# radygenomics/GROM

Measured on AMD Instinct MI355X. Metric: Mbases/sec scanned (whole genome) + VCF concordance vs ref, higher is better.
Workload: dtype int32

## Files before the change

grom_amd/csrc/ddecode.hip:

```cpp
#include <hip/hip_runtime.h>

#include <atomic>
#include <chrono>
#include <condition_variable>
#include <cstdio>
#include <cstdlib>
#include <cstring>
#include <mutex>
#include <vector>
#include <zlib.h>

#include "../../include/grom_amd.h"
#include "ddecode.h"
#include "inflate.h"

#define DD_LANES 64
#define DD_SLOTS 2
#define DD_RSLOTS 4

#define GI_E_BOUNDS 8
__device__ __forceinline__ bool dd_blk_inb(const DdBlock &b, int64_t o, int64_t comp_cap, int64_t out_cap) {
    return b.in_off >= 0 && b.in_off + (int64_t)b.in_len <= comp_cap && o >= 0 && b.out_len <= 65536u &&
           o + (int64_t)b.out_len <= out_cap;
}

__global__ void __launch_bounds__(DD_LANES, 2) k_inflate(const uint8_t *__restrict__ comp, int64_t comp_cap,
                                                      const DdBlock *__restrict__ blk, int64_t n_blk,
                                                      uint8_t *__restrict__ out, int64_t out_base, int64_t out_cap,
                                                      uint8_t *__restrict__ status, uint32_t *__restrict__ n_bad,
                                                      uint32_t *__restrict__ bounds, int only_tokcap) {
    extern __shared__ uint32_t dd_tab[];
    const int64_t j = (int64_t)blockIdx.x * DD_LANES + threadIdx.x;
    if (j >= n_blk) return;
    if (only_tokcap && status[j] != (uint8_t)GI_E_TOKCAP) return;
    const DdBlock b = blk[j];
    const int64_t o = b.out_off - out_base;
    if (!dd_blk_inb(b, o, comp_cap, out_cap)) {
        status[j] = (uint8_t)GI_E_BOUNDS;
        atomicAdd(n_bad, 1u);
        atomicOr(bounds, 1u);
        return;
    }
    const int rc = gi_inflate<DD_LANES>(comp + b.in_off, b.in_len, out + o, b.out_len, dd_tab, threadIdx.x);
    status[j] = (uint8_t)rc;
    if (rc) atomicAdd(n_bad, 1u);
}

__global__ void __launch_bounds__(DD_LANES, 2) k_huff(const uint8_t *__restrict__ comp, int64_t comp_cap,
                                                   const DdBlock *__restrict__ blk, int64_t n_blk,
                                                   uint8_t *__restrict__ out, int64_t out_base, int64_t out_cap,
                                                   uint32_t *__restrict__ tok, uint32_t *__restrict__ ntok,
                                                   uint32_t tokcap, uint8_t *__restrict__ status,
                                                   uint32_t *__restrict__ n_bad, uint32_t *__restrict__ bounds) {
    extern __shared__ uint32_t dd_tab[];
    const int64_t j = (int64_t)blockIdx.x * DD_LANES + threadIdx.x;
    if (j >= n_blk) return;
    const DdBlock b = blk[j];
    const int64_t o = b.out_off - out_base;
    if (!dd_blk_inb(b, o, comp_cap, out_cap)) {
        status[j] = (uint8_t)GI_E_BOUNDS;
        atomicAdd(n_bad, 1u);
        atomicOr(bounds, 1u);
        return;
    }
    const int rc = gi_tokens<DD_LANES>(comp + b.in_off, b.in_len, out + o, b.out_len, tok + (size_t)j * tokcap, tokcap,
                                       ntok + j, dd_tab, threadIdx.x);
    status[j] = (uint8_t)rc;
    if (rc && rc != GI_E_TOKCAP) atomicAdd(n_bad, 1u);
}

__device__ __forceinline__ uint32_t lz_wave_incl(uint32_t v, int lane) {
#pragma unroll
    for (int d = 1; d < 64; d <<= 1) {
        const uint32_t u = __shfl_up(v, d, 64);
        if (lane >= d) v += u;
    }
    return v;
}
__device__ __forceinline__ uint32_t lz_wave_min(uint32_t v) {
#pragma unroll
    for (int d = 32; d >= 1; d >>= 1) v = min(v, (uint32_t)__shfl_xor(v, d, 64));
    return v;
}

__global__ void __launch_bounds__(64) k_lz77(const DdBlock *__restrict__ blk, int64_t n_blk, uint8_t *__restrict__ out,
                                             int64_t out_base, const uint32_t *__restrict__ tok,
                                             const uint32_t *__restrict__ ntok, uint32_t tokcap,
                                             uint8_t *__restrict__ status, uint32_t *__restrict__ n_bad) {
    const int64_t j = blockIdx.x;
// ... 29 lines not shown
                bool blocked = false;
                for (uint64_t q = pm; q; q &= q - 1) {
                    const int jl = __builtin_ctzll(q);
                    const uint32_t mj = __builtin_amdgcn_readlane(m, jl);
                    const uint32_t ej = mj + __builtin_amdgcn_readlane(len, jl);
                    blocked = blocked || (mj < se && ej > src);
                }
                ready = pend && !blocked;
            }
            if (ready) {
                gi_match(dst, m, len, d);
                pend = false;
            }
            __builtin_amdgcn_fence(__ATOMIC_RELEASE, "workgroup");
            __builtin_amdgcn_fence(__ATOMIC_ACQUIRE, "workgroup");
        }
    }
    if (lane == 0 && (bad || obase != olen)) {
        status[j] = (uint8_t)GI_E_SIZE;
        atomicAdd(n_bad, 1u);
    }
}

__global__ void __launch_bounds__(DD_LANES) k_lz77_lane(const DdBlock *__restrict__ blk, int64_t n_blk,
                                                        uint8_t *__restrict__ out, int64_t out_base,
                                                        const uint32_t *__restrict__ tok,
                                                        const uint32_t *__restrict__ ntok, uint32_t tokcap,
                                                        uint8_t *__restrict__ status, uint32_t *__restrict__ n_bad) {
    const int64_t j = (int64_t)blockIdx.x * DD_LANES + threadIdx.x;
    if (j >= n_blk || status[j] != 0) return;
    const DdBlock b = blk[j];
    const int rc = gi_lz(tok + (size_t)j * tokcap, ntok[j], out + (b.out_off - out_base), b.out_len);
    if (rc) {
        status[j] = (uint8_t)rc;
        atomicAdd(n_bad, 1u);
    }
}

static uint32_t dd_tokcap() {
    static const uint32_t cap = [] {
        const char *e = getenv("GROM_INFLATE_TOKCAP");
        long v = e ? atol(e) : 0;
        if (v < 0) v = 0;
        if (v > 65536) v = 65536;
        return (uint32_t)(v & ~3L);
    }();
    return cap;
}

extern "C" size_t dd_inflate_tok_bytes(int64_t n_blk) {
    const uint32_t cap = dd_tokcap();
    return cap ? (size_t)n_blk * ((size_t)cap + 1) * 4 + 64 : 0;
}

extern "C" int dd_inflate_launch(hipStream_t st, const uint8_t *d_comp, int64_t comp_cap, const DdBlock *d_blk,
                                 int64_t n_blk, uint8_t *d_out, int64_t out_base, int64_t out_cap, uint8_t *d_status,
                                 uint32_t *d_bad, uint32_t *d_bounds, uint32_t *d_tok, size_t tok_bytes) {
    if (n_blk <= 0) return 0;
    const unsigned grid = (unsigned)((n_blk + DD_LANES - 1) / DD_LANES);
    static const int pad = getenv("GROM_INFLATE_LDS_PAD") ? atoi(getenv("GROM_INFLATE_LDS_PAD")) : 0;
    const uint32_t cap = dd_tokcap();
    if (cap == 0 || d_tok == nullptr || tok_bytes < dd_inflate_tok_bytes(n_blk)) {
        hipLaunchKernelGGL(k_inflate, dim3(grid), dim3(DD_LANES), GI_LANE_BYTES * DD_LANES + pad, st, d_comp, comp_cap,
                           d_blk, n_blk, d_out, out_base, out_cap, d_status, d_bad, d_bounds, 0);
        return hipGetLastError() == hipSuccess ? 0 : -1;
    }
    uint32_t *ntok = d_tok + (size_t)n_blk * cap;
    hipLaunchKernelGGL(k_huff, dim3(grid), dim3(DD_LANES), GI_LANE_BYTES * DD_LANES + pad, st, d_comp, comp_cap, d_blk,
                       n_blk, d_out, out_base, out_cap, d_tok, ntok, cap, d_status, d_bad, d_bounds);
    static const bool lane_lz = getenv("GROM_LZ_LANE") && atoi(getenv("GROM_LZ_LANE")) != 0;
    if (lane_lz)
        hipLaunchKernelGGL(k_lz77_lane, dim3(grid), dim3(DD_LANES), 0, st, d_blk, n_blk, d_out, out_base, d_tok, ntok,
                           cap, d_status, d_bad);
    else
        hipLaunchKernelGGL(k_lz77, dim3((unsigned)n_blk), dim3(64), 0, st, d_blk, n_blk, d_out, out_base, d_tok, ntok,
                           cap, d_status, d_bad);
    hipLaunchKernelGGL(k_inflate, dim3(grid), dim3(DD_LANES), GI_LANE_BYTES * DD_LANES + pad, st, d_comp, comp_cap,
                       d_blk, n_blk, d_out, out_base, out_cap, d_status, d_bad, d_bounds, 1);
    return hipGetLastError() == hipSuccess ? 0 : -1;
}

static uint16_t rd16(const uint8_t *p) { return (uint16_t)(p[0] | (p[1] << 8)); }
static uint32_t rd32(const uint8_t *p) {
    return (uint32_t)p[0] | (uint32_t)p[1] << 8 | (uint32_t)p[2] << 16 | (uint32_t)p[3] << 24;
}

extern "C" int64_t dd_block_table(const uint8_t *buf, int64_t len, DdBlock *out, int64_t cap, int64_t *out_bytes) {
    return dd_block_table_prefix(buf, len, out, cap, out_bytes, nullptr);
}

extern "C" int64_t dd_block_table_prefix(const uint8_t *buf, int64_t len, DdBlock *out, int64_t cap, int64_t *out_bytes,
                                         int64_t *consumed) {
    int64_t off = 0, n = 0, ob = 0;
    while (off < len) {
        if (off + 18 > len) {
            if (consumed) break;
            return -1;
        }
        const uint8_t *h = buf + off;
// ... 111 lines not shown
            inflateEnd(&zs);
            const bool same = zok ? (status[j] == 0 && memcmp(want.data(), got.data() + tab[j].out_off, tab[j].out_len) == 0)
                                  : status[j] != 0;
            if (!same) {
                if (bad < 5) fprintf(stderr, "device inflate: block %lld: zlib %d, device status %d\n", (long long)j, zrc,
                                     status[j]);
                bad++;
            }
        }
    }
done:
    if (n_blocks) *n_blocks = nb;
    if (bytes) *bytes = ob;
    if (e0) (void)hipEventDestroy(e0);
    if (e1) (void)hipEventDestroy(e1);
    if (st) (void)hipStreamDestroy(st);
    (void)hipFree(d_comp);
    (void)hipFree(d_out);
    (void)hipFree(d_status);
    (void)hipFree(d_blk);
    (void)hipFree(d_bad);
    (void)hipFree(d_tok);
    return bad;
}

#include <hipcub/hipcub.hpp>

#include "bamio.h"
#include "copystats.h"

namespace {

struct DBuf {
    void *p = nullptr;
    size_t cap = 0;
};

std::atomic<int64_t> g_dgrow_ns{0};

int dgrow(DBuf &b, size_t bytes, const char *what = nullptr) {
    if (bytes == 0) bytes = 16;
    if (b.cap >= bytes) return 0;
    const auto t0 = std::chrono::steady_clock::now();
    if (b.p) grom_dev_free(b.p, b.cap, GROM_DEVCAT_DECODE);
    b.p = nullptr;
    b.cap = 0;
// ... 1109 lines not shown
}

static int upload_run_tables(dd_ctx *c, const dd_run_req *q, hipStream_t st, char *err, int errlen) {
    const int64_t nblk = q->nblk, ns = q->n_starts;
    DBuf &rblk = c->rblk[q->slot], &rS = c->rS[q->slot];
    c->tab_gen[q->slot] = c->comp_gen[q->slot].load();
    DGROW(rblk, sizeof(DdBlock) * (size_t)(nblk + 1));
    DGROW(rS, sizeof(int64_t) * (size_t)(ns + 2));
    DCK(hipMemcpyAsync(rblk.p, q->blk, sizeof(DdBlock) * (size_t)nblk, hipMemcpyHostToDevice, st));
    DCK(hipMemcpyAsync(rS.p, q->starts, sizeof(int64_t) * (size_t)(ns + 1), hipMemcpyHostToDevice, st));
    return 0;
}

static int size_slot(RunSlot &r, const std::vector<Piece> &pcs, double rpb, char *err, int errlen) {
    int64_t mx_pb = 0, mx_blk = 0, mx_ch = 0, mx_oc = 0;
    for (const Piece &pc : pcs) {
        mx_pb = std::max(mx_pb, pc.pbytes);
        mx_blk = std::max(mx_blk, pc.bl - pc.bf + 2);
        mx_ch = std::max(mx_ch, pc.cb - pc.ca + 1);
        mx_oc = std::max(mx_oc, (int64_t)((double)pc.pbytes * rpb * 1.3) + 4096);
    }
    DGROW(r.U, (size_t)mx_pb + 64);
    DGROW(r.status, (size_t)mx_blk);
    DGROW(r.ccnt, sizeof(uint32_t) * (size_t)mx_ch);
    DGROW(r.cbase, sizeof(uint32_t) * (size_t)mx_ch);
    DGROW(r.misc, 256);
    DGROW(r.off, 8 * (size_t)(mx_oc + 1));
    size_t tb = 0;
    DCK(hipcub::DeviceScan::ExclusiveSum(nullptr, tb, (uint32_t *)nullptr, (uint32_t *)nullptr, (int)mx_ch, r.st));
    DGROW(r.tmp, tb);
    return 0;
}

__global__ void k_piece_summary(const uint32_t *__restrict__ cbase, const uint32_t *__restrict__ ccnt, int64_t nch,
                                uint32_t *__restrict__ rb, uint32_t *__restrict__ out) {
    if (threadIdx.x == 0) {
        out[0] = cbase[nch - 1];
        out[1] = ccnt[nch - 1];
        out[2] = rb[0];
        out[3] = rb[1];
        out[4] = rb[4];
        out[5] = rb[5];
    }
    __syncthreads();
    if (threadIdx.x < 16) rb[threadIdx.x] = 0;
}
// ... 507 lines not shown
```

grom_amd/csrc/inflate.h:

```cpp
#pragma once
#include <stdint.h>

#if defined(__HIP_DEVICE_COMPILE__)
#define GI_KEEP(x) asm volatile("" : "+v"(x))
#else
#define GI_KEEP(x) (void)0
#endif
#if defined(__HIPCC__)
#define GI_FN __host__ __device__ __forceinline__
#define GI_UNROLL _Pragma("unroll")
#else
#define GI_FN static inline
#define GI_UNROLL _Pragma("GCC unroll 16")
#endif

#define GI_T_LIT 0
#define GI_T_LITHI 72
#define GI_T_DIST 81
#ifndef GI_CLREG
#define GI_CLREG 0
#endif
#if GI_CLREG
#define GI_LANE_DWORDS 89
#else
// ... 104 lines not shown
        b.buf |= (uint64_t)b.q0 << b.cnt;
        b.q0 = b.q1;
        b.q1 = b.q2;
        b.q2 = b.q3;
        if (--b.kq == 0) {
            b.q0 = b.n0;
            b.q1 = b.n1;
            b.q2 = b.n2;
            b.q3 = b.n3;
            gi_ldq(b.wp, b.n0, b.n1, b.n2, b.n3);
            b.wp += 4;
            b.kq = 4;
        }
#else
        b.buf |= (uint64_t)b.nxt << b.cnt;
        b.nxt = gi_ldw(b.wp);
        b.wp++;
#endif
        b.cnt += 32;
        b.merged++;
    }
}

GI_FN uint32_t gi_bits(GiBits &b, int n) {
    const uint32_t v = (uint32_t)(b.buf & ((n >= 32) ? 0xffffffffull : ((1ull << n) - 1)));
    b.buf >>= n;
    b.cnt -= n;
    return v;
}

template <int LANES>
GI_FN uint8_t *gi_cell(uint32_t *tab, int t0, int r, int lane) {
    return (uint8_t *)(tab + (t0 + (r >> 2)) * LANES + lane) + (r & 3);
}

template <int N>
struct GiHuffT {
    uint32_t e[N + 1];
};
typedef GiHuffT<15> GiHuff;
typedef GiHuffT<7> GiHuffCL;

template <int N>
GI_FN int gi_code(GiHuffT<N> &h, uint32_t *cnt, int sh) {
    int32_t left = 1;
    uint32_t code = 0, off = 0;
GI_UNROLL
// ... 31 lines not shown
    }
}

template <int LANES, int N, bool HI, class Get>
GI_FN int gi_build(GiHuffT<N> &h, uint32_t *tab, int lane, int t0, int n, Get get) {
    uint32_t cnt[N + 1];
GI_UNROLL
    for (int l = 0; l <= N; l++) cnt[l] = 0;
    for (int i = 0; i < n; i++) {
        const uint32_t L = get(i);
GI_UNROLL
        for (int l = 1; l <= N; l++) cnt[l] += (L == (uint32_t)l) ? 1u : 0u;
    }
    const int rc = gi_code<N>(h, cnt, 0);
    if (rc) return rc;
    gi_clear_hi<LANES, HI>(tab, lane);
    for (int i = 0; i < n; i++) {
        const uint32_t L = get(i);
        if (L) gi_place<LANES, N, HI>(tab, t0, lane, cnt, 0, L, i);
    }
    return GI_OK;
}

template <int N>
GI_FN int gi_index(const GiBits &b, const GiHuffT<N> &h, int &L) {
    const uint32_t rev = gi_rev15((uint32_t)b.buf);
    const uint32_t key = rev << 16 | 0xffffu;
    L = 1;
    uint32_t bs = h.e[1];
GI_UNROLL
    for (int l = 1; l < N; l++) {
        const bool ge = key >= h.e[l];
        L += ge ? 1 : 0;
        bs = ge ? h.e[l + 1] : bs;
        GI_KEEP(bs);
    }
    if (key >= h.e[N]) return -1;
    return (int)(int16_t)(uint16_t)bs + (int)(rev >> (15 - L));
}

template <int LANES, int N, bool HI>
GI_FN int gi_lookup(const GiBits &b, const GiHuffT<N> &h, const uint32_t *tab, int lane, int t0, int &L) {
    const int idx = gi_index<N>(b, h, L);
    if (idx < 0) return -1;
    int s = *gi_cell<LANES>((uint32_t *)tab, t0, idx, lane);
    if (HI) s |= (int)((tab[(GI_T_LITHI + (idx >> 5)) * LANES + lane] >> (idx & 31)) & 1u) << 8;
    return s;
}

template <int LANES, int N, bool HI>
GI_FN int gi_decode(GiBits &b, const GiHuffT<N> &h, const uint32_t *tab, int lane, int t0) {
    int L;
    const int s = gi_lookup<LANES, N, HI>(b, h, tab, lane, t0, L);
    if (s < 0) return -1;
    b.buf >>= L;
    b.cnt -= L;
    return s;
}

GI_FN void gi_len_code(int s, int &base, int &extra) {
    if (s < 265) { base = s - 254; extra = 0; }
    else if (s < 285) { extra = (s - 261) >> 2; base = 3 + ((4 + ((s - 265) & 3)) << extra); }
    else { base = 258; extra = 0; }
}
GI_FN void gi_dist_code(int d, int &base, int &extra) {
    if (d < 4) { base = d + 1; extra = 0; }
    else { extra = (d >> 1) - 1; base = ((2 + (d & 1)) << extra) + 1; }
}

GI_FN int gi_cl_item(GiBits &b, int s, int prev, int &val) {
    if (s < 16) { val = s; return 1; }
    if (s == 16) { val = prev; return prev < 0 ? -1 : 3 + (int)gi_bits(b, 2); }
    val = 0;
    return s == 17 ? 3 + (int)gi_bits(b, 3) : 11 + (int)gi_bits(b, 7);
}

template <int LANES>
GI_FN int gi_fixed(GiHuff &lit, GiHuff &dist, uint32_t *tab, int lane) {
GI_UNROLL
    for (int w = 0; w < 72; w++) {
        uint32_t v = 0;
        for (int k = 0; k < 4; k++) {
            const int i = 4 * w + k;
            const int sym = i < 24 ? 256 + i : i < 168 ? i - 24 : i < 176 ? 280 + (i - 168) : 144 + (i - 176);
            v |= (uint32_t)(sym & 0xff) << (8 * k);
        }
        tab[(GI_T_LIT + w) * LANES + lane] = v;
    }
GI_UNROLL
    for (int w = 0; w < 9; w++) tab[(GI_T_LITHI + w) * LANES + lane] = w == 0 ? 0x00ffffffu : (w == 5 ? 0x0000ff00u : 0u);
GI_UNROLL
    for (int w = 0; w < 8; w++)
        tab[(GI_T_DIST + w) * LANES + lane] = (uint32_t)(4 * w) | (uint32_t)(4 * w + 1) << 8 | (uint32_t)(4 * w + 2) << 16 |
// ... 8 lines not shown

#ifndef GI_P2ONE
#define GI_P2ONE 1
#endif
struct GiHdr {
    GiHuffCL clh;
#if GI_CLREG
    uint32_t clt[4];
#endif
    int at;
    int n, ntot, nlit, prev, eob;
    int rl;
};

GI_FN void gi_seek(GiBits &b, const uint8_t *in, int pos) {
    const int mis = (int)((uintptr_t)in & 3);
    const int abs = mis * 8 + pos;
    b.sh0 = mis * 8;
    gi_start(b, (const uint32_t *)(in - mis), abs >> 5, abs & 31);
}

GI_FN int64_t gi_used(const GiBits &b) { return b.merged * 32 - b.sh0 - b.cnt; }

#if GI_CLREG
GI_FN int gi_build_cl(GiHdr &H, uint64_t cl) {
    uint32_t cnt[8];
GI_UNROLL
    for (int l = 0; l < 8; l++) cnt[l] = 0;
GI_UNROLL
    for (int i = 0; i < 19; i++) {
        const uint32_t L = (uint32_t)(cl >> (3 * i)) & 7u;
GI_UNROLL
        for (int l = 1; l <= 7; l++) cnt[l] += (L == (uint32_t)l) ? 1u : 0u;
    }
    const int rc = gi_code<7>(H.clh, cnt, 0);
    if (rc) return rc;
    H.clt[0] = H.clt[1] = H.clt[2] = H.clt[3] = 0;
GI_UNROLL
    for (int i = 0; i < 19; i++) {
        const uint32_t L = (uint32_t)(cl >> (3 * i)) & 7u;
        if (!L) continue;
        uint32_t o = 0;
GI_UNROLL
        for (int l = 1; l <= 7; l++) {
            o = (L == (uint32_t)l) ? cnt[l] : o;
            cnt[l] += (L == (uint32_t)l) ? 1u : 0u;
        }
        const uint32_t r = o / 6u, v = (uint32_t)i << (5u * (o - 6u * r));
        H.clt[0] |= r == 0 ? v : 0u;
        H.clt[1] |= r == 1 ? v : 0u;
        H.clt[2] |= r == 2 ? v : 0u;
        H.clt[3] |= r == 3 ? v : 0u;
    }
    return GI_OK;
}

GI_FN int gi_decode_cl(GiBits &b, const GiHdr &H) {
    int L;
    const int idx = gi_index<7>(b, H.clh, L);
    if (idx < 0) return -1;
    b.buf >>= L;
    b.cnt -= L;
    const uint32_t r = (uint32_t)idx / 6u;
    uint32_t w = H.clt[0];
    w = r == 1 ? H.clt[1] : w;
    GI_KEEP(w);
    w = r == 2 ? H.clt[2] : w;
    GI_KEEP(w);
    w = r == 3 ? H.clt[3] : w;
    return (int)((w >> (5u * ((uint32_t)idx - 6u * r))) & 31u);
}
#define GI_CL_DECODE(b, H) gi_decode_cl(b, H)
#else
#define GI_CL_DECODE(b, H) gi_decode<LANES, 7, false>(b, (H).clh, tab, lane, GI_T_CL)
#endif

template <int LANES>
GI_FN int gi_header(GiBits &b, GiHuff &lit, GiHuff &dist, GiHdr &H, uint32_t *tab, int lane, uint32_t &bfinal,
                    uint32_t &rem) {
    const uint32_t hdr = gi_bits(b, 3);
    bfinal = hdr & 1;
    const uint32_t btype = hdr >> 1;
    if (btype == 0) {
        gi_bits(b, b.cnt & 7);
        gi_refill(b);
        const uint32_t len = gi_bits(b, 16);
        gi_refill(b);
        const uint32_t nlen = gi_bits(b, 16);
        if ((len ^ 0xffffu) != nlen) return -GI_E_HEADER;
        rem = len;
        return len ? GI_M_STORED : (bfinal ? GI_M_DONE : GI_M_HDR);
    }
    if (btype == 1) {
        const int rc = gi_fixed<LANES>(lit, dist, tab, lane);
        return rc ? -rc : GI_M_SYM;
    }
    if (btype != 2) return -GI_E_HEADER;
    H.nlit = (int)gi_bits(b, 5) + 257;
    const int ndist = (int)gi_bits(b, 5) + 1;
    const int ncl = (int)gi_bits(b, 4) + 4;
    if (H.nlit > 286 || ndist > 30) return -GI_E_HEADER;
// ... 14 lines not shown
                                             [cl](int i) -> uint32_t { return (uint32_t)(cl >> (3 * i)) & 7u; });
#endif
    if (rc) return -rc;
    H.ntot = H.nlit + ndist;
    H.at = (int)gi_used(b);
GI_UNROLL
    for (int l = 0; l < 16; l++) lit.e[l] = 0;
    H.n = 0;
    H.prev = -1;
    H.eob = 0;
    return GI_M_P1;
}

GI_FN int gi_kraft(const uint32_t *cnt, int sh) {
    int32_t left = 1;
GI_UNROLL
    for (int l = 1; l <= 15; l++) {
        left = (left << 1) - (int32_t)((cnt[l] >> sh) & 0xffffu);
        if (left < 0) return GI_E_TREE;
    }
    return GI_OK;
}

template <int LANES, bool PASS2>
GI_FN int gi_cl_step(GiBits &b, const uint8_t *in, GiHuff &lit, GiHuff &dist, GiHdr &H, uint32_t *tab, int lane) {
    uint32_t *cn = lit.e;
#if GI_P2ONE
    if (PASS2) {
        if (H.rl == 0) {
            const int s = GI_CL_DECODE(b, H);
            if (s < 0) return -GI_E_TREE;
            int val;
            const int rep = gi_cl_item(b, s, H.prev, val);
            if (rep < 0 || H.n + rep > H.ntot) return -GI_E_TREE;
            H.prev = val;
            if (val) H.rl = rep;
            else H.n += rep;
        }
        if (H.rl > 0) {
            const int i = H.n;
            if (i < H.nlit) gi_place<LANES, 15, true>(tab, GI_T_LIT, lane, cn, 0, (uint32_t)H.prev, i);
            else gi_place<LANES, 15, false>(tab, GI_T_DIST, lane, cn, 16, (uint32_t)H.prev, i - H.nlit);
            H.n++;
            H.rl--;
        }
        if (H.n < H.ntot) return GI_M_P2;
        for (int l = 15; l >= 1; l--) cn[l] -= cn[l - 1];
        int rc = gi_code<15>(dist, cn, 16);
// ... 231 lines not shown
            if (!rem) mode = GI_M_SYM;
        } else if (mode == GI_M_STORED) {
            commit();
            gi_refill(b);
            const uint32_t m = rem < 4u ? rem : 4u;
            for (uint32_t j = 0; j < m; j++) gi_lit(out, o, pend, pn, gi_bits(b, 8));
            GI_BYTES(2, m);
            rem -= m;
            if (!rem) mode = bfinal ? GI_M_DONE : GI_M_HDR;
        }
    }
    if (rc) return rc;
    commit();
    gi_flush(out, o, out_len, pend, pn);
    const int64_t used_bits = gi_used(b);
    if (used_bits > 8 * (int64_t)in_len) return GI_E_INPUT;
    if (o != out_len) return GI_E_SIZE;
    return GI_OK;
}

enum { GI_E_TOKCAP = 9 };
#define GI_TOK_LITONLY 0x80000000u

template <int LANES>
GI_FN int gi_tokens(const uint8_t *in, uint32_t in_len, uint8_t *out, uint32_t out_len, uint32_t *tok, uint32_t tokcap,
                    uint32_t *ntok, uint32_t *tab, int lane) {
    typedef uint32_t gi_u32x4 __attribute__((vector_size(16)));
    GiBits b;
    gi_open(b, in);
    GiHuff lit_h = {}, dist_h = {};
    GiHdr H = {};
    uint32_t o = 0, bfinal = 0, rem = 0;
    uint64_t pend = 0;
    uint32_t pn = 0;
    uint32_t lc = 0;
    uint32_t nt = 0;
    gi_u32x4 tv = {};
    int mode = GI_M_HDR, rc = GI_OK;
    auto emit = [&](uint32_t t) -> bool {
        if (nt >= tokcap) return false;
        tv = (gi_u32x4){tv[1], tv[2], tv[3], t};
        nt++;
        if ((nt & 3u) == 0) __builtin_memcpy(tok + (nt - 4), &tv, 16);
        return true;
    };
    auto put_lit = [&](uint32_t s) -> bool {
        gi_lit(out, o, pend, pn, s);
        if (++lc == 255) {
            lc = 0;
            return emit(GI_TOK_LITONLY | 255u);
        }
        return true;
    };
    while (mode != GI_M_DONE) {
        GI_TRIP(mode);
        gi_refill(b);
        if (mode == GI_M_HDR) {
            const int m = gi_header<LANES>(b, lit_h, dist_h, H, tab, lane, bfinal, rem);
            if (m < 0) {
                rc = -m;
                break;
            }
            if (m == GI_M_STORED && o + rem > out_len) {
                rc = GI_E_OVERRUN;
                break;
            }
            mode = m;
        } else if (mode == GI_M_P1 || mode == GI_M_P2) {
            const int m = mode == GI_M_P1 ? gi_cl_step<LANES, false>(b, in, lit_h, dist_h, H, tab, lane)
                                          : gi_cl_step<LANES, true>(b, in, lit_h, dist_h, H, tab, lane);
            if (m < 0) {
                rc = -m;
                break;
            }
            mode = m;
        } else if (mode == GI_M_SYM) {
            const int s = gi_decode<LANES, 15, true>(b, lit_h, tab, lane, GI_T_LIT);
// ... 36 lines not shown
                }
                if (!emit(lc | (len - 3u) << 8 | (dd - 1u) << 16)) {
                    rc = GI_E_TOKCAP;
                    break;
                }
                lc = 0;
                gi_flush(out, o, out_len, pend, pn);
                o += len;
                GI_BYTES(1, len);
            }
        } else if (mode == GI_M_STORED) {
            const uint32_t m = rem < 4u ? rem : 4u;
            bool ok = true;
            for (uint32_t j = 0; j < m; j++) ok = put_lit(gi_bits(b, 8)) && ok;
            if (!ok) {
                rc = GI_E_TOKCAP;
                break;
            }
            GI_BYTES(2, m);
            rem -= m;
            if (!rem) mode = bfinal ? GI_M_DONE : GI_M_HDR;
        }
    }
    if (rc) return rc;
    if (lc && !emit(GI_TOK_LITONLY | lc)) return GI_E_TOKCAP;
    gi_flush(out, o, out_len, pend, pn);
    const uint32_t tail = nt & 3u;
    if (tail) {
        for (uint32_t k = tail; k < 4; k++) tv = (gi_u32x4){tv[1], tv[2], tv[3], 0u};
        __builtin_memcpy(tok + (nt - tail), &tv, 16);
    }
    *ntok = nt;
    const int64_t used_bits = gi_used(b);
    if (used_bits > 8 * (int64_t)in_len) return GI_E_INPUT;
    if (o != out_len) return GI_E_SIZE;
    return GI_OK;
}

GI_FN void gi_put_part(uint8_t *q, const uint32_t *w, uint32_t n) {
    uint32_t k = 0;
    if (n & 8) {
        const uint64_t v = (uint64_t)w[0] | (uint64_t)w[1] << 32;
        __builtin_memcpy(q, &v, 8);
        k = 2;
    }
    uint32_t x = w[k], y = w[k + 1];
// ... 63 lines not shown
```

grom_amd/csrc/inflate_host.cpp:

```cpp
#include <stdio.h>
#include <stdlib.h>
#include <string.h>
#include <zlib.h>

#include <vector>

#include "../../include/grom_amd.h"
#include "inflate.h"

extern "C" int grom_inflate_block_host(const uint8_t *in, uint32_t in_len, uint8_t *out, uint32_t out_len) {
    thread_local uint32_t tab[GI_LANE_DWORDS];
    return gi_inflate<1>(in, in_len, out, out_len, tab, 0);
}

extern "C" int grom_inflate_block_host2(const uint8_t *in, uint32_t in_len, uint8_t *out, uint32_t out_len,
                                        uint32_t tokcap) {
    thread_local uint32_t tab[GI_LANE_DWORDS];
    thread_local std::vector<uint32_t> tok;
    tok.assign(((size_t)tokcap + 3) & ~(size_t)3, 0);
    uint32_t nt = 0;
    const int rc = gi_tokens<1>(in, in_len, out, out_len, tok.data(), tokcap & ~3u, &nt, tab, 0);
    return rc ? rc : gi_lz(tok.data(), nt, out, out_len);
}

static uint16_t rd16(const uint8_t *p) { return (uint16_t)(p[0] | (p[1] << 8)); }
static uint32_t rd32(const uint8_t *p) { return (uint32_t)p[0] | (uint32_t)p[1] << 8 | (uint32_t)p[2] << 16 | (uint32_t)p[3] << 24; }

extern "C" int64_t grom_inflate_selftest(const char *bam_path, int64_t max_blocks, int64_t *n_blocks, int64_t *bytes) {
    FILE *f = fopen(bam_path, "rb");
    if (!f) return -1;
    fseek(f, 0, SEEK_END);
    const long size = ftell(f);
    fseek(f, 0, SEEK_SET);
    std::vector<uint8_t> file((size_t)size + 64);
    if (fread(file.data(), 1, (size_t)size, f) != (size_t)size) {
        fclose(f);
        return -1;
    }
    fclose(f);
    std::vector<uint8_t> a(65536 + 64), b(65536 + 64);
    int64_t bad = 0, nb = 0, nbytes = 0;
    long off = 0;
    while (off + 18 <= size && (max_blocks <= 0 || nb < max_blocks)) {
        const uint8_t *h = file.data() + off;
// ... 7 lines not shown
        }
        if (bsize < 0 || off + bsize + 1 > size) return -3;
        const long blen = bsize + 1;
        const uint32_t isize = rd32(h + blen - 4);
        const uint8_t *data = h + 12 + xlen;
        const uint32_t dlen = (uint32_t)(blen - 12 - xlen - 8);
        if (isize > 65536) return -4;
        z_stream zs;
        memset(&zs, 0, sizeof(zs));
        int zrc = inflateInit2(&zs, -15);
        zs.next_in = (Bytef *)data;
        zs.avail_in = dlen;
        zs.next_out = a.data();
        zs.avail_out = (uInt)a.size();
        if (zrc == Z_OK) zrc = inflate(&zs, Z_FINISH);
        const bool zok = zrc == Z_STREAM_END && zs.total_out == isize;
        inflateEnd(&zs);
        memset(b.data(), 0xa5, b.size());
        const int rc = grom_inflate_block_host(data, dlen, b.data(), isize);
        bool same = zok ? (rc == GI_OK && memcmp(a.data(), b.data(), isize) == 0) : (rc != GI_OK);
        memset(b.data(), 0x5a, b.size());
        const int rc2 = grom_inflate_block_host2(data, dlen, b.data(), isize, 65536);
        same = same && (zok ? (rc2 == GI_OK && memcmp(a.data(), b.data(), isize) == 0) : (rc2 != GI_OK));
        if (!same) {
            if (bad < 5) fprintf(stderr, "inflate selftest: block at %ld (isize %u): zlib %d, twin %d\n", off, isize, zrc, rc);
            bad++;
        }
        nbytes += isize;
        nb++;
        off += blen;
    }
    if (n_blocks) *n_blocks = nb;
    if (bytes) *bytes = nbytes;
    return bad;
}
```

Measured before the change: 895.0.

## Add LDS-ring bit reader for Huffman pass and LDS-staged LZ77 kernel

Adds an optional ring-buffer bit reader that prefetches compressed words into LDS through 16-byte vector loads, serviced every few decode trips, so the Huffman token pass hides global-load latency. Also adds an optional LZ77 kernel that stages each 64 KiB output block into LDS, resolves matches there with vectorised copies, and writes the block back, replacing scattered global byte copies. Both paths are gated behind environment variables that default to off. The token buffer is now also allocated in the reusable resources, and host and device self-tests were added.

```diff
diff --git a/grom_amd/csrc/ddecode.hip b/grom_amd/csrc/ddecode.hip
--- a/grom_amd/csrc/ddecode.hip
+++ b/grom_amd/csrc/ddecode.hip
@@ -46,6 +46,7 @@
     if (rc) atomicAdd(n_bad, 1u);
 }
 
+template <bool RING>
 __global__ void __launch_bounds__(DD_LANES, 2) k_huff(const uint8_t *__restrict__ comp, int64_t comp_cap,
                                                    const DdBlock *__restrict__ blk, int64_t n_blk,
                                                    uint8_t *__restrict__ out, int64_t out_base, int64_t out_cap,
@@ -63,8 +64,10 @@
         atomicOr(bounds, 1u);
         return;
     }
-    const int rc = gi_tokens<DD_LANES>(comp + b.in_off, b.in_len, out + o, b.out_len, tok + (size_t)j * tokcap, tokcap,
-                                       ntok + j, dd_tab, threadIdx.x);
+    const int64_t room = comp_cap - b.in_off;
+    const int rc = gi_tokens<DD_LANES, RING>(comp + b.in_off, b.in_len,
+                                             (uint32_t)(room < 0x7fffffff ? room : 0x7fffffff), out + o, b.out_len,
+                                             tok + (size_t)j * tokcap, tokcap, ntok + j, dd_tab, threadIdx.x);
     status[j] = (uint8_t)rc;
     if (rc && rc != GI_E_TOKCAP) atomicAdd(n_bad, 1u);
 }
@@ -140,6 +143,139 @@
     }
 }
 
+#define LZ_THREADS 256
+#define LZ_LDS_BYTES (65536 + 48)
+
+__device__ __forceinline__ void lz_copy(uint8_t *w, uint32_t o, uint32_t rem, uint32_t D) {
+    while (rem) {
+        const uint32_t lim = rem < 16u ? rem : 16u;
+        const uint32_t c = lim < D ? lim : D;
+        const uint8_t *s = w + (o - D);
+        uint8_t *q = w + o;
+        uint32_t v[4];
+        __builtin_memcpy(v, s, 16);
+        if (lim == 16u) {
+            __builtin_memcpy(q, v, 16);
+        } else {
+            uint32_t k = 0;
+            if (lim & 8u) {
+                __builtin_memcpy(q, v, 8);
+                k = 2;
+            }
+            uint32_t x = k ? v[2] : v[0];
+            const uint32_t y = k ? v[3] : v[1];
+            if (lim & 4u) {
+                __builtin_memcpy(q + (lim & 8u), &x, 4);
+                x = y;
+            }
+            const uint32_t at = lim & 12u;
+            if (lim & 2u) {
+                const uint16_t h = (uint16_t)x;
+                __builtin_memcpy(q + at, &h, 2);
+                x >>= 16;
+            }
+            if (lim & 1u) q[at + (lim & 2u)] = (uint8_t)x;
+        }
+        o += c;
+        rem -= c;
+        if (c == D && D < 16u) D <<= 1;
+    }
+}
+
+template <bool IN>
+__device__ __forceinline__ void lz_stage(uint8_t *w, uint8_t *g, uint32_t olen, uint32_t tid) {
+    typedef uint32_t lz_q4 __attribute__((ext_vector_type(4)));
+    uint32_t h = (16u - (uint32_t)((uintptr_t)g & 15u)) & 15u;
+    h = h < olen ? h : olen;
+    const uint32_t nq = (olen - h) >> 4, t0 = h + 16u * nq;
+    if (tid < h) {
+        if (IN) w[tid] = g[tid];
+        else g[tid] = w[tid];
+    }
+    for (uint32_t q = tid; q < nq; q += LZ_THREADS) {
+        if (IN) *(lz_q4 *)(w + h + 16u * q) = *(const lz_q4 *)(g + h + 16u * q);
+        else *(lz_q4 *)(g + h + 16u * q) = *(const lz_q4 *)(w + h + 16u * q);
+    }
+    if (tid < olen - t0) {
+        if (IN) w[t0 + tid] = g[t0 + tid];
+        else g[t0 + tid] = w[t0 + tid];
+    }
+}
+
+__global__ void __launch_bounds__(LZ_THREADS) k_lz77_lds(const DdBlock *__restrict__ blk, int64_t n_blk, uint8_t *out,
+                                                         int64_t out_base, const uint32_t *__restrict__ tok,
+                                                         const uint32_t *__restrict__ ntok, uint32_t tokcap,
+                                                         uint8_t *__restrict__ status, uint32_t *__restrict__ n_bad) {
+    extern __shared__ __attribute__((aligned(16))) uint8_t lz_lds[];
+    __shared__ int lz_bad;
+    const int64_t j = blockIdx.x;
+    if (j >= n_blk || status[j] != 0) return;
+    const uint32_t tid = threadIdx.x;
+    const DdBlock b = blk[j];
+    const uint32_t olen = b.out_len;
+    if (olen == 0 || olen > 65536u) return;
+    uint8_t *dst = out + (b.out_off - out_base);
+    uint8_t *w = lz_lds + ((uintptr_t)dst & 15u);
+    if (tid == 0) lz_bad = 0;
+    lz_stage<true>(w, dst, olen, tid);
+    __syncthreads();
+    if (tid < 64) {
+        const int lane = (int)tid;
+        const uint32_t n = ntok[j];
+        const uint32_t *tk = tok + (size_t)j * tokcap;
+        uint32_t obase = 0;
+        bool bad = n > tokcap;
+        uint32_t tn = (!bad && (uint32_t)lane < n) ? tk[lane] : GI_TOK_LITONLY;
+        for (uint32_t c0 = 0; c0 < n && !bad; c0 += 64) {
+            const uint32_t t = tn;
+            const uint32_t kn = c0 + 64u + (uint32_t)lane;
+            tn = kn < n ? tk[kn] : GI_TOK_LITONLY;
+            const bool hm = !(t & GI_TOK_LITONLY);
+            const uint32_t lc = t & 255u, len = hm ? ((t >> 8) & 255u) + 3u : 0u, d = ((t >> 16) & 0x7fffu) + 1u;
+            const uint32_t span = lc + len;
+            const uint32_t inc = lz_wave_incl(span, lane);
+            const uint32_t m = obase + inc - len;
+            obase += __shfl(inc, 63, 64);
+            bool pend = hm;
+            if (__any((hm && d > m) || obase > olen)) {
+                bad = true;
+                break;
+            }
+            const uint32_t src = m - d, se = src + (len < d ? len : d);
+            for (;;) {
+                const uint64_t pm = __ballot(pend);
+                if (pm == 0) break;
+                const uint32_t P = lz_wave_min(pend ? m : 0xffffffffu);
+                bool ready = pend && se <= P;
+                if (__ballot(ready) != pm) {
+                    bool blocked = false;
+                    for (uint64_t q = pm; q; q &= q - 1) {
+                        const int jl = __builtin_ctzll(q);
+                        const uint32_t mj = __builtin_amdgcn_readlane(m, jl);
+                        const uint32_t ej = mj + __builtin_amdgcn_readlane(len, jl);
+                        blocked = blocked || (mj < se && ej > src);
+                    }
+                    ready = pend && !blocked;
+                }
+                if (ready) {
+                    lz_copy(w, m, len, d);
+                    pend = false;
+                }
+                __builtin_amdgcn_fence(__ATOMIC_RELEASE, "wavefront");
+                __builtin_amdgcn_fence(__ATOMIC_ACQUIRE, "wavefront");
+            }
+        }
+        if (lane == 0 && (bad || obase != olen)) {
+            lz_bad = 1;
+            status[j] = (uint8_t)GI_E_SIZE;
+            atomicAdd(n_bad, 1u);
+        }
+    }
+    __syncthreads();
+    if (lz_bad) return;
+    lz_stage<false>(w, dst, olen, tid);
+}
+
 __global__ void __launch_bounds__(DD_LANES) k_lz77_lane(const DdBlock *__restrict__ blk, int64_t n_blk,
                                                         uint8_t *__restrict__ out, int64_t out_base,
                                                         const uint32_t *__restrict__ tok,
@@ -184,15 +320,34 @@
         return hipGetLastError() == hipSuccess ? 0 : -1;
     }
     uint32_t *ntok = d_tok + (size_t)n_blk * cap;
-    hipLaunchKernelGGL(k_huff, dim3(grid), dim3(DD_LANES), GI_LANE_BYTES * DD_LANES + pad, st, d_comp, comp_cap, d_blk,
-                       n_blk, d_out, out_base, out_cap, d_tok, ntok, cap, d_status, d_bad, d_bounds);
+    static const bool ring = getenv("GROM_HUFF_RING") && atoi(getenv("GROM_HUFF_RING")) != 0;
+    if (ring)
+        hipLaunchKernelGGL(k_huff<true>, dim3(grid), dim3(DD_LANES), GI_TOK_LANE_BYTES * DD_LANES + pad, st, d_comp,
+                           comp_cap, d_blk, n_blk, d_out, out_base, out_cap, d_tok, ntok, cap, d_status, d_bad, d_bounds);
+    else
+        hipLaunchKernelGGL(k_huff<false>, dim3(grid), dim3(DD_LANES), GI_LANE_BYTES * DD_LANES + pad, st, d_comp,
+                           comp_cap, d_blk, n_blk, d_out, out_base, out_cap, d_tok, ntok, cap, d_status, d_bad, d_bounds);
     static const bool lane_lz = getenv("GROM_LZ_LANE") && atoi(getenv("GROM_LZ_LANE")) != 0;
+    static const bool lds_lz = getenv("GROM_LZ_LDS") && atoi(getenv("GROM_LZ_LDS")) != 0;
     if (lane_lz)
         hipLaunchKernelGGL(k_lz77_lane, dim3(grid), dim3(DD_LANES), 0, st, d_blk, n_blk, d_out, out_base, d_tok, ntok,
                            cap, d_status, d_bad);
-    else
+    else if (!lds_lz)
         hipLaunchKernelGGL(k_lz77, dim3((unsigned)n_blk), dim3(64), 0, st, d_blk, n_blk, d_out, out_base, d_tok, ntok,
                            cap, d_status, d_bad);
+    else {
+        static std::atomic<bool> lds_set[64];
+        int dev = 0;
+        if (hipGetDevice(&dev) != hipSuccess || dev < 0 || dev >= 64) return -1;
+        if (!lds_set[dev].load(std::memory_order_acquire)) {
+            if (hipFuncSetAttribute((const void *)k_lz77_lds, hipFuncAttributeMaxDynamicSharedMemorySize, LZ_LDS_BYTES) !=
+                hipSuccess)
+                return -1;
+            lds_set[dev].store(true, std::memory_order_release);
+        }
+        hipLaunchKernelGGL(k_lz77_lds, dim3((unsigned)n_blk), dim3(LZ_THREADS), LZ_LDS_BYTES, st, d_blk, n_blk, d_out,
+                           out_base, d_tok, ntok, cap, d_status, d_bad);
+    }
     hipLaunchKernelGGL(k_inflate, dim3(grid), dim3(DD_LANES), GI_LANE_BYTES * DD_LANES + pad, st, d_comp, comp_cap,
                        d_blk, n_blk, d_out, out_base, out_cap, d_status, d_bad, d_bounds, 1);
     return hipGetLastError() == hipSuccess ? 0 : -1;
@@ -350,6 +505,91 @@
     (void)hipFree(d_bad);
     (void)hipFree(d_tok);
     return bad;
+}
+
+extern "C" int64_t grom_inflate_device_guard_selftest(const char *bgzf_path, int device, int64_t *n_blocks,
+                                                      int64_t *n_stray) {
+    FILE *f = fopen(bgzf_path, "rb");
+    if (!f) return -1;
+    fseek(f, 0, SEEK_END);
+    const int64_t size = ftell(f);
+    fseek(f, 0, SEEK_SET);
+    std::vector<uint8_t> file((size_t)size + 64, 0);
+    if (fread(file.data(), 1, (size_t)size, f) != (size_t)size) { fclose(f); return -1; }
+    fclose(f);
+    int64_t ob = 0;
+    const int64_t nb = dd_block_table(file.data(), size, nullptr, 0, &ob);
+    if (nb <= 0) return -2;
+    std::vector<DdBlock> tab((size_t)nb);
+    dd_block_table(file.data(), size, tab.data(), nb, &ob);
+    int64_t cur = 0;
+    for (int64_t j = 0; j < nb; j++) {
+        cur += ((j & 15) - cur) & 15;
+        tab[j].out_off = cur;
+        cur += (int64_t)tab[j].out_len + 48;
+    }
+    const int64_t total = cur + 16;
+    if (hipSetDevice(device) != hipSuccess) return -3;
+    uint8_t *d_comp = nullptr, *d_out = nullptr, *d_status = nullptr;
+    DdBlock *d_blk = nullptr;
+    uint32_t *d_bad = nullptr, *d_tok = nullptr;
+    const size_t tok_bytes = dd_inflate_tok_bytes(nb);
+    int64_t bad = -4, stray = 0;
+    hipStream_t st = nullptr;
+    if (hipMalloc(&d_comp, (size_t)size + 64) != hipSuccess || hipMalloc(&d_out, (size_t)total) != hipSuccess ||
+        hipMalloc(&d_status, (size_t)nb + 1) != hipSuccess || hipMalloc(&d_blk, sizeof(DdBlock) * (size_t)(nb + 1)) != hipSuccess ||
+        hipMalloc(&d_bad, 8) != hipSuccess || (tok_bytes && hipMalloc(&d_tok, tok_bytes) != hipSuccess) ||
+        hipStreamCreate(&st) != hipSuccess || ((uintptr_t)d_out & 15u) != 0)
+        goto done;
+    {
+        (void)hipMemcpyAsync(d_comp, file.data(), (size_t)size + 64, hipMemcpyHostToDevice, st);
+        (void)hipMemcpyAsync(d_blk, tab.data(), sizeof(DdBlock) * (size_t)nb, hipMemcpyHostToDevice, st);
+        (void)hipMemsetAsync(d_bad, 0, 8, st);
+        (void)hipMemsetAsync(d_out, 0xA5, (size_t)total, st);
+        if (dd_inflate_launch(st, d_comp, size + 64, d_blk, nb, d_out, 0, total, d_status, d_bad, d_bad + 1, d_tok, tok_bytes))
+            goto done;
+        if (hipStreamSynchronize(st) != hipSuccess) goto done;
+        std::vector<uint8_t> got((size_t)total), status((size_t)nb);
+        if (hipMemcpy(got.data(), d_out, (size_t)total, hipMemcpyDeviceToHost) != hipSuccess ||
+            hipMemcpy(status.data(), d_status, (size_t)nb, hipMemcpyDeviceToHost) != hipSuccess)
+            goto done;
+        bad = 0;
+        std::vector<uint8_t> want(65536 + 64);
+        int64_t prev_end = 0;
+        for (int64_t j = 0; j <= nb; j++) {
+            const int64_t lo = j < nb ? tab[j].out_off : total;
+            for (int64_t i = prev_end; i < lo; i++) stray += got[(size_t)i] != 0xA5;
+            if (j == nb) break;
+            prev_end = lo + tab[j].out_len;
+            z_stream zs;
+            memset(&zs, 0, sizeof(zs));
+            int zrc = inflateInit2(&zs, -15);
+            zs.next_in = (Bytef *)(file.data() + tab[j].in_off);
+            zs.avail_in = tab[j].in_len;
+            zs.next_out = want.data();
+            zs.avail_out = (uInt)want.size();
+            if (zrc == Z_OK) zrc = inflate(&zs, Z_FINISH);
+            const bool zok = zrc == Z_STREAM_END && zs.total_out == tab[j].out_len;
+            inflateEnd(&zs);
+            if (!(zok && status[j] == 0 && memcmp(want.data(), got.data() + lo, tab[j].out_len) == 0)) {
+                if (bad < 5) fprintf(stderr, "device inflate guard: block %lld (%u bytes): zlib %d, device status %d\n",
+                                     (long long)j, tab[j].out_len, zrc, status[j]);
+                bad++;
+            }
+        }
+        if (stray) fprintf(stderr, "device inflate guard: %lld bytes outside the blocks overwritten\n", (long long)stray);
+    }
+done:
+    if (n_blocks) *n_blocks = nb;
+    if (n_stray) *n_stray = stray;
+    if (st) (void)hipStreamDestroy(st);
+    (void)hipFree(d_comp);
+    (void)hipFree(d_out);
+    (void)hipFree(d_status);
+    (void)hipFree(d_blk);
+    (void)hipFree(d_bad);
+    (void)hipFree(d_tok);
+    return bad < 0 ? bad : bad + stray;
 }
 
 #include <hipcub/hipcub.hpp>
@@ -1505,6 +1745,7 @@
     }
     DGROW(r.U, (size_t)mx_pb + 64);
     DGROW(r.status, (size_t)mx_blk);
+    if (dd_inflate_tok_bytes(1)) DGROW(r.tok, dd_inflate_tok_bytes(mx_blk));
     DGROW(r.ccnt, sizeof(uint32_t) * (size_t)mx_ch);
     DGROW(r.cbase, sizeof(uint32_t) * (size_t)mx_ch);
     DGROW(r.misc, 256);
diff --git a/grom_amd/csrc/inflate.h b/grom_amd/csrc/inflate.h
--- a/grom_amd/csrc/inflate.h
+++ b/grom_amd/csrc/inflate.h
@@ -150,7 +150,8 @@
     }
 }
 
-GI_FN uint32_t gi_bits(GiBits &b, int n) {
+template <class B>
+GI_FN uint32_t gi_bits(B &b, int n) {
     const uint32_t v = (uint32_t)(b.buf & ((n >= 32) ? 0xffffffffull : ((1ull << n) - 1)));
     b.buf >>= n;
     b.cnt -= n;
@@ -228,8 +229,8 @@
     return GI_OK;
 }
 
-template <int N>
-GI_FN int gi_index(const GiBits &b, const GiHuffT<N> &h, int &L) {
+template <int N, class B>
+GI_FN int gi_index(const B &b, const GiHuffT<N> &h, int &L) {
     const uint32_t rev = gi_rev15((uint32_t)b.buf);
     const uint32_t key = rev << 16 | 0xffffu;
     L = 1;
@@ -245,8 +246,8 @@
     return (int)(int16_t)(uint16_t)bs + (int)(rev >> (15 - L));
 }
 
-template <int LANES, int N, bool HI>
-GI_FN int gi_lookup(const GiBits &b, const GiHuffT<N> &h, const uint32_t *tab, int lane, int t0, int &L) {
+template <int LANES, int N, bool HI, class B>
+GI_FN int gi_lookup(const B &b, const GiHuffT<N> &h, const uint32_t *tab, int lane, int t0, int &L) {
     const int idx = gi_index<N>(b, h, L);
     if (idx < 0) return -1;
     int s = *gi_cell<LANES>((uint32_t *)tab, t0, idx, lane);
@@ -254,8 +255,8 @@
     return s;
 }
 
-template <int LANES, int N, bool HI>
-GI_FN int gi_decode(GiBits &b, const GiHuffT<N> &h, const uint32_t *tab, int lane, int t0) {
+template <int LANES, int N, bool HI, class B>
+GI_FN int gi_decode(B &b, const GiHuffT<N> &h, const uint32_t *tab, int lane, int t0) {
     int L;
     const int s = gi_lookup<LANES, N, HI>(b, h, tab, lane, t0, L);
     if (s < 0) return -1;
@@ -274,7 +275,8 @@
     else { extra = (d >> 1) - 1; base = ((2 + (d & 1)) << extra) + 1; }
 }
 
-GI_FN int gi_cl_item(GiBits &b, int s, int prev, int &val) {
+template <class B>
+GI_FN int gi_cl_item(B &b, int s, int prev, int &val) {
     if (s < 16) { val = s; return 1; }
     if (s == 16) { val = prev; return prev < 0 ? -1 : 3 + (int)gi_bits(b, 2); }
     val = 0;
@@ -329,6 +331,153 @@
 
 GI_FN int64_t gi_used(const GiBits &b) { return b.merged * 32 - b.sh0 - b.cnt; }
 
+#define GI_RING_WORDS 32
+#define GI_RING_NEED 4u
+#define GI_SERVICE_TRIPS 2u
+#define GI_T_RING GI_LANE_DWORDS
+#define GI_TOK_LANE_DWORDS (GI_LANE_DWORDS + GI_RING_WORDS)
+#define GI_TOK_LANE_BYTES (GI_TOK_LANE_DWORDS * 4)
+#if defined(__HIP_DEVICE_COMPILE__)
+#define GI_UNIFORM(x) ((uint32_t)__builtin_amdgcn_readfirstlane((int)(x)))
+#else
+#define GI_UNIFORM(x) (x)
+#endif
+
+template <int LANES>
+struct GiRing {
+    uint64_t buf;
+    int cnt;
+    int sh0;
+    int skip;
+    uint32_t *ring;
+    const uint32_t *base;
+    uint32_t lim;
+    uint32_t rd, wr, ld;
+    uint32_t s0, s1, s2, s3;
+};
+
+template <int LANES>
+GI_FN uint32_t gi_ring_word(const GiRing<LANES> &b, uint32_t i) {
+    if (4u * i + 4u <= b.lim) return gi_ldw(b.base + i);
+    uint32_t v = 0;
+    for (uint32_t t = 0; t < 4; t++)
+        if (4u * i + t < b.lim) v |= (uint32_t)((const uint8_t *)b.base)[4u * i + t] << (8u * t);
+    return v;
+}
+
+template <int LANES>
+GI_FN void gi_seek(GiRing<LANES> &b, const uint8_t *, int pos) {
+    const int abs = b.sh0 + pos;
+    b.rd = b.wr = b.ld = (uint32_t)(abs >> 5);
+    b.skip = abs & 31;
+    b.buf = 0;
+    b.cnt = 0;
+}
+
+template <int LANES>
+GI_FN void gi_ring_open(GiRing<LANES> &b, const uint8_t *in, uint32_t in_len, uint32_t in_room, uint32_t *tab,
+                        int lane) {
+    const int mis = (int)((uintptr_t)in & 3);
+    b.sh0 = mis * 8;
+    b.ring = tab + GI_T_RING * LANES + lane;
+    b.base = (const uint32_t *)(in - mis);
+    const uint32_t past = in_room <= in_len ? 0u : (in_room - in_len < 8u ? in_room - in_len : 8u);
+    b.lim = (uint32_t)mis + in_len + past;
+    b.s0 = b.s1 = b.s2 = b.s3 = 0;
+    gi_seek(b, in, 0);
+}
+
+template <int LANES>
+GI_FN void gi_service(GiRing<LANES> &b) {
+    if (b.ld != b.wr && b.wr - b.rd + 4u <= GI_RING_WORDS) {
+        uint32_t w0 = b.s0, w1 = b.s1, w2 = b.s2, w3 = b.s3;
+        if (4u * b.wr + 16u > b.lim) {
+            w0 = w1 = w2 = w3 = 0;
+            if (4u * b.wr < b.lim) {
+                w0 = gi_ring_word(b, b.wr);
+                w1 = gi_ring_word(b, b.wr + 1);
+                w2 = gi_ring_word(b, b.wr + 2);
+                w3 = gi_ring_word(b, b.wr + 3);
+            }
+        }
+        b.ring[((b.wr + 0u) & (GI_RING_WORDS - 1)) * LANES] = w0;
+        b.ring[((b.wr + 1u) & (GI_RING_WORDS - 1)) * LANES] = w1;
+        b.ring[((b.wr + 2u) & (GI_RING_WORDS - 1)) * LANES] = w2;
+        b.ring[((b.wr + 3u) & (GI_RING_WORDS - 1)) * LANES] = w3;
+        b.wr += 4;
+    }
+    if (b.ld == b.wr) {
+        if (4u * b.ld + 16u <= b.lim) {
+#if defined(__HIP_DEVICE_COMPILE__)
+            typedef uint32_t gi_q4 __attribute__((ext_vector_type(4), aligned(4)));
+            const gi_q4 v = *(const gi_q4 *)(b.base + b.ld);
+            b.s0 = v.x;
+            b.s1 = v.y;
+            b.s2 = v.z;
+            b.s3 = v.w;
+#else
+            b.s0 = gi_ldw(b.base + b.ld);
+            b.s1 = gi_ldw(b.base + b.ld + 1);
+            b.s2 = gi_ldw(b.base + b.ld + 2);
+            b.s3 = gi_ldw(b.base + b.ld + 3);
+#endif
+        }
+        b.ld += 4;
+    }
+}
+
+template <int LANES>
+GI_FN void gi_refill(GiRing<LANES> &b) {
+    if (b.cnt < 32) {
+        b.buf |= (uint64_t)b.ring[(b.rd & (GI_RING_WORDS - 1)) * LANES] << b.cnt;
+        b.rd++;
+        b.cnt += 32;
+    }
+}
+
+template <int LANES>
+GI_FN void gi_ring_prime(GiRing<LANES> &b) {
+    b.buf = (uint64_t)(b.ring[(b.rd & (GI_RING_WORDS - 1)) * LANES] >> b.skip);
+    b.cnt = 32 - b.skip;
+    b.rd++;
+    b.skip = -1;
+    gi_refill(b);
+}
+
+template <int LANES>
+GI_FN int64_t gi_used(const GiRing<LANES> &b) {
+    return (int64_t)b.rd * 32 - b.sh0 - b.cnt + (b.skip > 0 ? b.skip : 0);
+}
+
+template <int LANES>
+GI_FN bool gi_trip_top(GiRing<LANES> &b, uint32_t trip, uint32_t &idle) {
+    if ((GI_UNIFORM(trip) & (GI_SERVICE_TRIPS - 1u)) == 0) gi_service<LANES>(b);
+    if (b.wr - b.rd < GI_RING_NEED) {
+        idle++;
+        return true;
+    }
+    if (b.skip >= 0) {
+        gi_ring_prime<LANES>(b);
+        return true;
+    }
+    return false;
+}
+GI_FN bool gi_trip_top(GiBits &, uint32_t, uint32_t &) { return false; }
+
+template <int LANES, bool RING>
+struct GiTokReader {
+    typedef GiBits type;
+};
+template <int LANES>
+struct GiTokReader<LANES, true> {
+    typedef GiRing<LANES> type;
+};
+GI_FN void gi_tok_open(GiBits &b, const uint8_t *in, uint32_t, uint32_t, uint32_t *, int) { gi_open(b, in); }
+template <int LANES>
+GI_FN void gi_tok_open(GiRing<LANES> &b, const uint8_t *in, uint32_t in_len, uint32_t in_room, uint32_t *tab, int lane) {
+    gi_ring_open<LANES>(b, in, in_len, in_room, tab, lane);
+}
+
 #if GI_CLREG
 GI_FN int gi_build_cl(GiHdr &H, uint64_t cl) {
     uint32_t cnt[8];
@@ -362,7 +511,8 @@
     return GI_OK;
 }
 
-GI_FN int gi_decode_cl(GiBits &b, const GiHdr &H) {
+template <class B>
+GI_FN int gi_decode_cl(B &b, const GiHdr &H) {
     int L;
     const int idx = gi_index<7>(b, H.clh, L);
     if (idx < 0) return -1;
@@ -382,8 +532,8 @@
 #define GI_CL_DECODE(b, H) gi_decode<LANES, 7, false>(b, (H).clh, tab, lane, GI_T_CL)
 #endif
 
-template <int LANES>
-GI_FN int gi_header(GiBits &b, GiHuff &lit, GiHuff &dist, GiHdr &H, uint32_t *tab, int lane, uint32_t &bfinal,
+template <int LANES, class B>
+GI_FN int gi_header(B &b, GiHuff &lit, GiHuff &dist, GiHdr &H, uint32_t *tab, int lane, uint32_t &bfinal,
                     uint32_t &rem) {
     const uint32_t hdr = gi_bits(b, 3);
     bfinal = hdr & 1;
@@ -444,8 +594,8 @@
     return GI_OK;
 }
 
-template <int LANES, bool PASS2>
-GI_FN int gi_cl_step(GiBits &b, const uint8_t *in, GiHuff &lit, GiHuff &dist, GiHdr &H, uint32_t *tab, int lane) {
+template <int LANES, bool PASS2, class B>
+GI_FN int gi_cl_step(B &b, const uint8_t *in, GiHuff &lit, GiHuff &dist, GiHdr &H, uint32_t *tab, int lane) {
     uint32_t *cn = lit.e;
 #if GI_P2ONE
     if (PASS2) {
@@ -723,12 +873,13 @@
 enum { GI_E_TOKCAP = 9 };
 #define GI_TOK_LITONLY 0x80000000u
 
-template <int LANES>
-GI_FN int gi_tokens(const uint8_t *in, uint32_t in_len, uint8_t *out, uint32_t out_len, uint32_t *tok, uint32_t tokcap,
-                    uint32_t *ntok, uint32_t *tab, int lane) {
+template <int LANES, bool RING = false>
+GI_FN int gi_tokens(const uint8_t *in, uint32_t in_len, uint32_t in_room, uint8_t *out, uint32_t out_len, uint32_t *tok,
+                    uint32_t tokcap, uint32_t *ntok, uint32_t *tab, int lane, uint32_t *idle_trips = nullptr) {
     typedef uint32_t gi_u32x4 __attribute__((vector_size(16)));
-    GiBits b;
-    gi_open(b, in);
+    typename GiTokReader<LANES, RING>::type b;
+    gi_tok_open(b, in, in_len, in_room, tab, lane);
+    uint32_t trip = 0, idle = 0;
     GiHuff lit_h = {}, dist_h = {};
     GiHdr H = {};
     uint32_t o = 0, bfinal = 0, rem = 0;
@@ -754,6 +905,7 @@
         return true;
     };
     while (mode != GI_M_DONE) {
+        if (gi_trip_top(b, trip++, idle)) continue;
         GI_TRIP(mode);
         gi_refill(b);
         if (mode == GI_M_HDR) {
@@ -836,6 +988,7 @@
             if (!rem) mode = bfinal ? GI_M_DONE : GI_M_HDR;
         }
     }
+    if (idle_trips) *idle_trips = idle;
     if (rc) return rc;
     if (lc && !emit(GI_TOK_LITONLY | lc)) return GI_E_TOKCAP;
     gi_flush(out, o, out_len, pend, pn);
diff --git a/grom_amd/csrc/inflate_host.cpp b/grom_amd/csrc/inflate_host.cpp
--- a/grom_amd/csrc/inflate_host.cpp
+++ b/grom_amd/csrc/inflate_host.cpp
@@ -13,13 +13,28 @@
     return gi_inflate<1>(in, in_len, out, out_len, tab, 0);
 }
 
+extern "C" int grom_inflate_block_host_ring(const uint8_t *in, uint32_t in_len, uint32_t in_room, uint8_t *out,
+                                            uint32_t out_len, uint32_t tokcap, uint32_t *n_tok, uint32_t *idle_trips);
+
 extern "C" int grom_inflate_block_host2(const uint8_t *in, uint32_t in_len, uint8_t *out, uint32_t out_len,
                                         uint32_t tokcap) {
     thread_local uint32_t tab[GI_LANE_DWORDS];
     thread_local std::vector<uint32_t> tok;
     tok.assign(((size_t)tokcap + 3) & ~(size_t)3, 0);
     uint32_t nt = 0;
-    const int rc = gi_tokens<1>(in, in_len, out, out_len, tok.data(), tokcap & ~3u, &nt, tab, 0);
+    const int rc = gi_tokens<1>(in, in_len, in_len + 8, out, out_len, tok.data(), tokcap & ~3u, &nt, tab, 0);
+    return rc ? rc : gi_lz(tok.data(), nt, out, out_len);
+}
+
+extern "C" int grom_inflate_block_host_ring(const uint8_t *in, uint32_t in_len, uint32_t in_room, uint8_t *out,
+                                            uint32_t out_len, uint32_t tokcap, uint32_t *n_tok, uint32_t *idle_trips) {
+    thread_local uint32_t tab[GI_TOK_LANE_DWORDS];
+    thread_local std::vector<uint32_t> tok;
+    tok.assign(((size_t)tokcap + 3) & ~(size_t)3, 0);
+    uint32_t nt = 0, idle = 0;
+    const int rc = gi_tokens<1, true>(in, in_len, in_room, out, out_len, tok.data(), tokcap & ~3u, &nt, tab, 0, &idle);
+    if (n_tok) *n_tok = nt;
+    if (idle_trips) *idle_trips = idle;
     return rc ? rc : gi_lz(tok.data(), nt, out, out_len);
 }
 
@@ -73,6 +88,9 @@
         memset(b.data(), 0x5a, b.size());
         const int rc2 = grom_inflate_block_host2(data, dlen, b.data(), isize, 65536);
         same = same && (zok ? (rc2 == GI_OK && memcmp(a.data(), b.data(), isize) == 0) : (rc2 != GI_OK));
+        memset(b.data(), 0x3c, b.size());
+        const int rc3 = grom_inflate_block_host_ring(data, dlen, dlen + 8, b.data(), isize, 65536, nullptr, nullptr);
+        same = same && (zok ? (rc3 == GI_OK && memcmp(a.data(), b.data(), isize) == 0) : (rc3 != GI_OK));
         if (!same) {
             if (bad < 5) fprintf(stderr, "inflate selftest: block at %ld (isize %u): zlib %d, twin %d\n", off, isize, zrc, rc);
             bad++;
```

Result: slower. 816.0 (-8.8%).
